# liruihui/SP-GAN

Measured on AMD Instinct MI355X. Metric: G+D train-step shapes/sec @2048 pts, bs=32 per GPU (WGAN-GP), higher is better.
Workload: dtype f32; 1 GPU; BASELINE configs[1]: Chair-shaped synthetic clouds, 2048 pts, per-GPU batch 32, WGAN + gradient penalty (lambda 10), 1 D-step + 1 G-step, Adam(1e-4, (0.5,0.99)), k=10; one latent per shape (default noise_generator) handed over un-tiled [b,1,128]; global_batch=32, n_points=2048, parallelism=dp1

## Files before the change

sp-gan_amd/csrc/sparse_rows.hpp:

```cpp
#pragma once
#include "common.hpp"

__device__ __forceinline__ void sparse_rows_nt_body(int bx, int b, unsigned* sm_u, const float* __restrict__ val, const int32_t* __restrict__ arg, int rows,
                                                    int Cs, const float* __restrict__ W, int ldw, int N, float* __restrict__ E, int lde, int RB) {
  const int words = (Cs + 63) / 64;
  unsigned* mask = sm_u;
  float* sval = reinterpret_cast<float*>(sm_u + RB * 2 * words);
  const int tid = threadIdx.x, lane = tid & 63, wave = tid >> 6;
  const int r0 = bx * RB;
  for (int i = tid; i < RB * 2 * words; i += 256) mask[i] = 0u;
  __syncthreads();
  for (int c = tid; c < Cs; c += 256) {
    sval[c] = val[(size_t)b * Cs + c];
    const int r = arg[(size_t)b * Cs + c] - b * rows - r0;
    if (r >= 0 && r < RB) atomicOr(&mask[r * 2 * words + (c >> 5)], 1u << (c & 31));
  }
  __syncthreads();
  for (int rl = wave; rl < RB && r0 + rl < rows; rl += 4) {
    float* e = E + ((size_t)b * rows + r0 + rl) * lde;
    const unsigned long long* mrow = reinterpret_cast<const unsigned long long*>(mask + rl * 2 * words);
    for (int n0 = 0; n0 < N; n0 += 256) {
      const int n = n0 + lane * 4;
      const bool vec = n0 + 256 <= N && (ldw & 3) == 0 && (reinterpret_cast<uintptr_t>(W) & 15) == 0;
      float4 acc = make_float4(0.f, 0.f, 0.f, 0.f);
      for (int w0 = 0; w0 < words; w0 += 64) {
        const unsigned long long mine = (w0 + lane < words) ? mrow[w0 + lane] : 0ull;
        unsigned long long nz = __ballot(mine != 0ull);
        while (nz) {
          const int wl = __ffsll((long long)nz) - 1;
          nz &= nz - 1;
          unsigned long long bits = __shfl(mine, wl);
          if (vec) {
            while (bits) {
              int cc[8];
              float4 wv[8];
#pragma unroll
              for (int u = 0; u < 8; ++u) {
                cc[u] = bits ? (w0 + wl) * 64 + __ffsll((long long)bits) - 1 : -1;
                bits &= bits - 1;
              }
#pragma unroll
              for (int u = 0; u < 8; ++u) wv[u] = *reinterpret_cast<const float4*>(W + (size_t)max(cc[u], 0) * ldw + n);
#pragma unroll
              for (int u = 0; u < 8; ++u) {
                if (cc[u] >= 0) {
                  const float v = sval[cc[u]];
                  acc.x = fmaf(v, wv[u].x, acc.x); acc.y = fmaf(v, wv[u].y, acc.y); acc.z = fmaf(v, wv[u].z, acc.z); acc.w = fmaf(v, wv[u].w, acc.w);
                }
              }
            }
          }
          while (bits) {
            const int cc = (w0 + wl) * 64 + __ffsll((long long)bits) - 1;
            bits &= bits - 1;
            const float v = sval[cc];
            const float* w = W + (size_t)cc * ldw + n;
            if (n + 3 < N) {
              acc.x = fmaf(v, w[0], acc.x); acc.y = fmaf(v, w[1], acc.y); acc.z = fmaf(v, w[2], acc.z); acc.w = fmaf(v, w[3], acc.w);
            } else {
              if (n < N) acc.x = fmaf(v, w[0], acc.x);
              if (n + 1 < N) acc.y = fmaf(v, w[1], acc.y);
              if (n + 2 < N) acc.z = fmaf(v, w[2], acc.z);
            }
          }
        }
      }
      if (n + 3 < N && (lde & 3) == 0 && (reinterpret_cast<uintptr_t>(E) & 15) == 0) {
        *reinterpret_cast<float4*>(e + n) = acc;
      } else {
        if (n < N) e[n] = acc.x;
        if (n + 1 < N) e[n + 1] = acc.y;
        if (n + 2 < N) e[n + 2] = acc.z;
        if (n + 3 < N) e[n + 3] = acc.w;
      }
    }
  }
}


static inline int sparse_rows_nt_rb(int rows, int Cs) {
  const int words = cdiv(Cs, 64);
  int RB = (32 * 1024) / (words * 8);
  if (RB > 32) RB = 32;
  if (RB > rows) RB = rows;
  return RB;
}
static inline size_t sparse_rows_nt_lds(int RB, int Cs) { return (size_t)RB * cdiv(Cs, 64) * 8 + (size_t)Cs * 4; }
```

Measured before the change: 3716 shapes/s.

## Interleave 8 rows per wave in sparse-row gather kernel to raise memory-level parallelism

Restructures the sparse row-gather GEMM so that each wave handles up to 8 output rows at once, keeping 8 float4 accumulators. For each row it issues the first weight-row load up front, so the loads of all rows are in flight together, then handles any remaining set bits per row. It also batches the val/arg loads into registers ahead of the LDS mask build, and uses readlane in place of shfl to broadcast mask words. This targets latency-bound serial gathers when each row has few nonzeros, at the cost of more registers and more complex control flow.

Result: no change. 3740 shapes/s (median of 6 runs) (+0.6%).

```diff
diff --git a/sp-gan_amd/csrc/sparse_rows.hpp b/sp-gan_amd/csrc/sparse_rows.hpp
--- a/sp-gan_amd/csrc/sparse_rows.hpp
+++ b/sp-gan_amd/csrc/sparse_rows.hpp
@@ -1,5 +1,27 @@
 #pragma once
 #include "common.hpp"
+
+constexpr int SR_WAVE_ROWS = 8;
+constexpr int SR_RB_MAX = 4 * SR_WAVE_ROWS;
+constexpr int SR_BATCH = 8;
+
+__device__ __forceinline__ unsigned long long sr_readlane64(unsigned long long v, int src) {
+  const unsigned lo = (unsigned)__builtin_amdgcn_readlane((int)(unsigned)v, src);
+  const unsigned hi = (unsigned)__builtin_amdgcn_readlane((int)(unsigned)(v >> 32), src);
+  return ((unsigned long long)hi << 32) | lo;
+}
+
+__device__ __forceinline__ float4 sr_row4(const float* __restrict__ row, unsigned n) { return *reinterpret_cast<const float4*>(row + n); }
+
+__device__ __forceinline__ void sr_fma_tail(float4& acc, float v, const float* __restrict__ w, int n, int N) {
+  if (n + 3 < N) {
+    acc.x = fmaf(v, w[0], acc.x); acc.y = fmaf(v, w[1], acc.y); acc.z = fmaf(v, w[2], acc.z); acc.w = fmaf(v, w[3], acc.w);
+  } else {
+    if (n < N) acc.x = fmaf(v, w[0], acc.x);
+    if (n + 1 < N) acc.y = fmaf(v, w[1], acc.y);
+    if (n + 2 < N) acc.z = fmaf(v, w[2], acc.z);
+  }
+}
 
 __device__ __forceinline__ void sparse_rows_nt_body(int bx, int b, unsigned* sm_u, const float* __restrict__ val, const int32_t* __restrict__ arg, int rows,
                                                     int Cs, const float* __restrict__ W, int ldw, int N, float* __restrict__ E, int lde, int RB) {
@@ -8,70 +30,136 @@
   float* sval = reinterpret_cast<float*>(sm_u + RB * 2 * words);
   const int tid = threadIdx.x, lane = tid & 63, wave = tid >> 6;
   const int r0 = bx * RB;
-  for (int i = tid; i < RB * 2 * words; i += 256) mask[i] = 0u;
-  __syncthreads();
-  for (int c = tid; c < Cs; c += 256) {
-    sval[c] = val[(size_t)b * Cs + c];
-    const int r = arg[(size_t)b * Cs + c] - b * rows - r0;
-    if (r >= 0 && r < RB) atomicOr(&mask[r * 2 * words + (c >> 5)], 1u << (c & 31));
+  const float* vb = val + (size_t)b * Cs;
+  const int32_t* ab = arg + (size_t)b * Cs;
+  for (int c0 = 0; c0 < Cs; c0 += 1024) {
+    int ar[4];
+    float vv[4];
+#pragma unroll
+    for (int i = 0; i < 4; ++i) {
+      const int c = c0 + tid + 256 * i;
+      ar[i] = c < Cs ? ab[c] : -1;
+      vv[i] = c < Cs ? vb[c] : 0.f;
+    }
+    if (c0 == 0) {
+      for (int i = tid; i < RB * 2 * words; i += 256) mask[i] = 0u;
+      __syncthreads();
+    }
+#pragma unroll
+    for (int i = 0; i < 4; ++i) {
+      const int c = c0 + tid + 256 * i;
+      if (c < Cs) {
+        sval[c] = vv[i];
+        const int r = ar[i] - b * rows - r0;
+        if (r >= 0 && r < RB) atomicOr(&mask[r * 2 * words + (c >> 5)], 1u << (c & 31));
+      }
+    }
   }
   __syncthreads();
-  for (int rl = wave; rl < RB && r0 + rl < rows; rl += 4) {
-    float* e = E + ((size_t)b * rows + r0 + rl) * lde;
-    const unsigned long long* mrow = reinterpret_cast<const unsigned long long*>(mask + rl * 2 * words);
-    for (int n0 = 0; n0 < N; n0 += 256) {
-      const int n = n0 + lane * 4;
-      const bool vec = n0 + 256 <= N && (ldw & 3) == 0 && (reinterpret_cast<uintptr_t>(W) & 15) == 0;
-      float4 acc = make_float4(0.f, 0.f, 0.f, 0.f);
-      for (int w0 = 0; w0 < words; w0 += 64) {
-        const unsigned long long mine = (w0 + lane < words) ? mrow[w0 + lane] : 0ull;
-        unsigned long long nz = __ballot(mine != 0ull);
-        while (nz) {
-          const int wl = __ffsll((long long)nz) - 1;
-          nz &= nz - 1;
-          unsigned long long bits = __shfl(mine, wl);
+  const bool vec_w = (ldw & 3) == 0 && (reinterpret_cast<uintptr_t>(W) & 15) == 0;
+  const bool vec_e = (lde & 3) == 0 && (reinterpret_cast<uintptr_t>(E) & 15) == 0;
+  for (int n0 = 0; n0 < N; n0 += 256) {
+    const int n = n0 + lane * 4;
+    const unsigned un = (unsigned)n;
+    const bool vec = n0 + 256 <= N && vec_w;
+    float4 acc[SR_WAVE_ROWS];
+#pragma unroll
+    for (int u = 0; u < SR_WAVE_ROWS; ++u) acc[u] = make_float4(0.f, 0.f, 0.f, 0.f);
+    for (int w0 = 0; w0 < words; w0 += 64) {
+      int c1[SR_WAVE_ROWS];
+      float4 w1[SR_WAVE_ROWS];
+      unsigned more = 0u;
+#pragma unroll
+      for (int u = 0; u < SR_WAVE_ROWS; ++u) {
+        const int rl = wave + 4 * u;
+        const bool live = rl < RB && r0 + rl < rows && w0 + lane < words;
+        const unsigned long long mine = live ? reinterpret_cast<const unsigned long long*>(mask + rl * 2 * words)[w0 + lane] : 0ull;
+        const unsigned long long nz = __ballot(mine != 0ull);
+        c1[u] = -1;
+        if (nz) {
+          if (vec) {
+            const int wl = __ffsll((long long)nz) - 1;
+            const unsigned long long bits = sr_readlane64(mine, wl);
+            c1[u] = (w0 + wl) * 64 + __ffsll((long long)bits) - 1;
+            w1[u] = sr_row4(W + (size_t)c1[u] * ldw, un);
+            if ((bits & (bits - 1)) | (nz & (nz - 1))) more |= 1u << u;
+          } else {
+            more |= 1u << u;
+          }
+        }
+      }
+#pragma unroll
+      for (int u = 0; u < SR_WAVE_ROWS; ++u) {
+        if (c1[u] >= 0) {
+          const float v = sval[c1[u]];
+          acc[u].x = fmaf(v, w1[u].x, acc[u].x); acc[u].y = fmaf(v, w1[u].y, acc[u].y); acc[u].z = fmaf(v, w1[u].z, acc[u].z); acc[u].w = fmaf(v, w1[u].w, acc[u].w);
+        }
+      }
+      while (more) {
+        const int u = __ffs((int)more) - 1;
+        more &= more - 1;
+        const int rl = wave + 4 * u;
+        const unsigned long long mine = w0 + lane < words ? reinterpret_cast<const unsigned long long*>(mask + rl * 2 * words)[w0 + lane] : 0ull;
+        unsigned long long left = __ballot(mine != 0ull);
+        bool first = vec;
+        float4 a = acc[0];
+#pragma unroll
+        for (int j = 1; j < SR_WAVE_ROWS; ++j)
+          if (u == j) a = acc[j];
+        while (left) {
+          const int wl = __ffsll((long long)left) - 1;
+          left &= left - 1;
+          unsigned long long bits = sr_readlane64(mine, wl);
+          if (first) {
+            bits &= bits - 1;
+            first = false;
+          }
           if (vec) {
             while (bits) {
-              int cc[8];
-              float4 wv[8];
+              int cc[SR_BATCH];
+              float4 wv[SR_BATCH];
 #pragma unroll
-              for (int u = 0; u < 8; ++u) {
-                cc[u] = bits ? (w0 + wl) * 64 + __ffsll((long long)bits) - 1 : -1;
+              for (int j = 0; j < SR_BATCH; ++j) {
+                cc[j] = bits ? (w0 + wl) * 64 + __ffsll((long long)bits) - 1 : -1;
                 bits &= bits - 1;
               }
 #pragma unroll
-              for (int u = 0; u < 8; ++u) wv[u] = *reinterpret_cast<const float4*>(W + (size_t)max(cc[u], 0) * ldw + n);
+              for (int j = 0; j < SR_BATCH; ++j)
+                if (cc[j] >= 0) wv[j] = sr_row4(W + (size_t)cc[j] * ldw, un);
 #pragma unroll
-              for (int u = 0; u < 8; ++u) {
-                if (cc[u] >= 0) {
-                  const float v = sval[cc[u]];
-                  acc.x = fmaf(v, wv[u].x, acc.x); acc.y = fmaf(v, wv[u].y, acc.y); acc.z = fmaf(v, wv[u].z, acc.z); acc.w = fmaf(v, wv[u].w, acc.w);
+              for (int j = 0; j < SR_BATCH; ++j) {
+                if (cc[j] >= 0) {
+                  const float v = sval[cc[j]];
+                  a.x = fmaf(v, wv[j].x, a.x); a.y = fmaf(v, wv[j].y, a.y); a.z = fmaf(v, wv[j].z, a.z); a.w = fmaf(v, wv[j].w, a.w);
                 }
               }
             }
-          }
-          while (bits) {
-            const int cc = (w0 + wl) * 64 + __ffsll((long long)bits) - 1;
-            bits &= bits - 1;
-            const float v = sval[cc];
-            const float* w = W + (size_t)cc * ldw + n;
-            if (n + 3 < N) {
-              acc.x = fmaf(v, w[0], acc.x); acc.y = fmaf(v, w[1], acc.y); acc.z = fmaf(v, w[2], acc.z); acc.w = fmaf(v, w[3], acc.w);
-            } else {
-              if (n < N) acc.x = fmaf(v, w[0], acc.x);
-              if (n + 1 < N) acc.y = fmaf(v, w[1], acc.y);
-              if (n + 2 < N) acc.z = fmaf(v, w[2], acc.z);
+          } else {
+            while (bits) {
+              const int cc = (w0 + wl) * 64 + __ffsll((long long)bits) - 1;
+              bits &= bits - 1;
+              sr_fma_tail(a, sval[cc], W + (size_t)cc * ldw + n, n, N);
             }
           }
         }
+#pragma unroll
+        for (int j = 0; j < SR_WAVE_ROWS; ++j)
+          if (u == j) acc[j] = a;
       }
-      if (n + 3 < N && (lde & 3) == 0 && (reinterpret_cast<uintptr_t>(E) & 15) == 0) {
-        *reinterpret_cast<float4*>(e + n) = acc;
-      } else {
-        if (n < N) e[n] = acc.x;
-        if (n + 1 < N) e[n + 1] = acc.y;
-        if (n + 2 < N) e[n + 2] = acc.z;
-        if (n + 3 < N) e[n + 3] = acc.w;
+    }
+#pragma unroll
+    for (int u = 0; u < SR_WAVE_ROWS; ++u) {
+      const int rl = wave + 4 * u;
+      if (rl < RB && r0 + rl < rows) {
+        float* e = E + ((size_t)b * rows + r0 + rl) * lde;
+        if (n + 3 < N && vec_e) {
+          *reinterpret_cast<float4*>(e + n) = acc[u];
+        } else {
+          if (n < N) e[n] = acc[u].x;
+          if (n + 1 < N) e[n + 1] = acc[u].y;
+          if (n + 2 < N) e[n + 2] = acc[u].z;
+          if (n + 3 < N) e[n + 3] = acc[u].w;
+        }
       }
     }
   }
@@ -81,7 +169,7 @@
 static inline int sparse_rows_nt_rb(int rows, int Cs) {
   const int words = cdiv(Cs, 64);
   int RB = (32 * 1024) / (words * 8);
-  if (RB > 32) RB = 32;
+  if (RB > SR_RB_MAX) RB = SR_RB_MAX;
   if (RB > rows) RB = rows;
   return RB;
 }
```
